# AIML-IfI/openset-imagenet

Measured on AMD Instinct MI355X. Metric: images/sec (whole node) ResNet-50 + entropic-open-set, Protocol 2, 1/2/4/8 GPUs, higher is better.
Workload: dtype f32; 1 GPU; Protocol 2, ResNet-50, entropic open-set loss, batch 128/GPU; workload_key=p2, classes=30, batch_per_gpu=128, global_batch=128, image=3x224x224, loss=entropic, optimizer=adam lr=1e-3, parallelism=dp1

## Files before the change

### openset-imagenet_amd/csrc/conv_wino.hip

```cpp
#include "conv_common.h"
#include <algorithm>
#include <type_traits>
#include <utility>

using namespace osi_conv;

namespace {

#ifndef OSI_WABL
#define OSI_WABL 0
#endif
#ifndef OSI_FABL
#define OSI_FABL 0
#endif
#ifndef OSI_STAGE_OUT
#define OSI_STAGE_OUT 1
#endif
#ifndef OSI_XSPREAD
#define OSI_XSPREAD 8
#endif
constexpr int KC = 16;
constexpr int PF = 6;

struct WinoP {
    const float* x;
    const float* u;
    float* y;
    const float* sc;
    const float* sh;
    int H, W, Kc, Nc, TH, TW, T, KS, CB, MT, NT;
    int x_bytes, y_bytes, u_bytes;
    float* pmean;
    float* pm2;
    int P;
    float cnt, rcnt;
    const float* ey0;
    const float *escale0, *eshift0, *emean0, *einv0;
    float* esum;
    const float *osc, *osh;
    int orelu;
    int q, r, nfull;
    float* slab;
    int slab_bytes;
};

__device__ __forceinline__ f32x2 pk_add(f32x2 a, f32x2 b) {
    f32x2 r;
    asm volatile("v_pk_add_f32 %0, %1, %2" : "=v"(r) : "v"(a), "v"(b));
    return r;
}
__device__ __forceinline__ f32x2 pk_sub(f32x2 a, f32x2 b) {
    f32x2 r;
    asm volatile("v_pk_add_f32 %0, %1, %2 neg_lo:[0,1] neg_hi:[0,1]" : "=v"(r) : "v"(a), "v"(b));
    return r;
}
__device__ __forceinline__ f32x2 pk_neg(f32x2 a) {
    f32x2 r;
    asm volatile("v_pk_add_f32 %0, 0, %1 neg_lo:[0,1] neg_hi:[0,1]" : "=v"(r) : "v"(a));
    return r;
}
__device__ __forceinline__ f32x2 pk_fma(f32x2 a, f32x2 b, f32x2 c) {
    f32x2 r;
    asm volatile("v_pk_fma_f32 %0, %1, %2, %3" : "=v"(r) : "v"(a), "v"(b), "v"(c));
    return r;
}
__device__ __forceinline__ f32x4 pk_add(f32x4 a, f32x4 b) {
    const f32x2 lo = pk_add(__builtin_shufflevector(a, a, 0, 1), __builtin_shufflevector(b, b, 0, 1));
    const f32x2 hi = pk_add(__builtin_shufflevector(a, a, 2, 3), __builtin_shufflevector(b, b, 2, 3));
    return __builtin_shufflevector(lo, hi, 0, 1, 2, 3);
}
__device__ __forceinline__ f32x4 pk_sub(f32x4 a, f32x4 b) {
    const f32x2 lo = pk_sub(__builtin_shufflevector(a, a, 0, 1), __builtin_shufflevector(b, b, 0, 1));
    const f32x2 hi = pk_sub(__builtin_shufflevector(a, a, 2, 3), __builtin_shufflevector(b, b, 2, 3));
    return __builtin_shufflevector(lo, hi, 0, 1, 2, 3);
}

template <class F, int... I>
__device__ __forceinline__ void for_each_const(F& f, std::integer_sequence<int, I...>) {
    (f(std::integral_constant<int, I>{}), ...);
}

__device__ __forceinline__ float row16_sum(float v) {
    v += __builtin_bit_cast(float, __builtin_amdgcn_update_dpp(0, __builtin_bit_cast(int, v), 0xB1, 0xF, 0xF, true));
    v += __builtin_bit_cast(float, __builtin_amdgcn_update_dpp(0, __builtin_bit_cast(int, v), 0x4E, 0xF, 0xF, true));
    v += __builtin_bit_cast(float, __builtin_amdgcn_update_dpp(0, __builtin_bit_cast(int, v), 0x141, 0xF, 0xF, true));
    v += __builtin_bit_cast(float, __builtin_amdgcn_update_dpp(0, __builtin_bit_cast(int, v), 0x140, 0xF, 0xF, true));
    return v;
}

template <int FLIP>
__global__ __launch_bounds__(256) void k_wino_weights(const float* __restrict__ w, float* __restrict__ u, int Kc, int Nc, int KS, int CB) {
    const int idx = blockIdx.x * 256 + threadIdx.x;
    const int K4 = Kc / 4;
    if (idx >= K4 * Nc) return;
    const int n = idx % Nc, k0 = (idx / Nc) * 4;
    f32x4 g[3][3];
#pragma unroll
    for (int r = 0; r < 3; ++r)
#pragma unroll
        for (int s = 0; s < 3; ++s) {
            if (FLIP) {
#pragma unroll
                for (int e = 0; e < 4; ++e) g[r][s][e] = w[((size_t)((k0 + e) * 3 + (2 - r)) * 3 + (2 - s)) * Nc + n];
            } else g[r][s] = ld4(w + ((size_t)(n * 3 + r) * 3 + s) * Kc + k0);
        }
    f32x4 t[4][3];
#pragma unroll
    for (int s = 0; s < 3; ++s) {
        t[0][s] = g[0][s];
        t[1][s] = 0.5f * (g[0][s] + g[1][s] + g[2][s]);
        t[2][s] = 0.5f * (g[0][s] - g[1][s] + g[2][s]);
        t[3][s] = g[2][s];
    }
    const int ks = k0 / KC, j = (k0 % KC) / 8, h = (k0 % 8) / 4, cb = n / 32, lane = h * 32 + n % 32;
#pragma unroll
    for (int xi = 0; xi < 4; ++xi) {
        f32x4 v[4];
        v[0] = t[xi][0];
        v[1] = 0.5f * (t[xi][0] + t[xi][1] + t[xi][2]);
        v[2] = 0.5f * (t[xi][0] - t[xi][1] + t[xi][2]);
        v[3] = t[xi][2];
#pragma unroll
        for (int nu = 0; nu < 4; ++nu) {
            const int p = xi * 4 + nu;
            *reinterpret_cast<f32x4*>(u + ((((size_t)(p * KS + ks) * CB + cb) * 2 + j) * 64 + lane) * 4) = v[nu];
        }
    }
}

struct Seg { int v, ks0, ks1, slot; bool valid; };

__device__ __forceinline__ void unit_of(int v, int MT, int NT, int& mt, int& nt) {
    const int full = (MT / 8) * 8 * NT;
    if (v < full) {
        const int xcd = v & 7, slot = v >> 3;
        nt = slot % NT;
        mt = (slot / NT) * 8 + xcd;
    } else {
        const int rem = MT & 7, vv = v - full;
        mt = (MT / 8) * 8 + vv % rem;
        nt = vv / rem;
    }
}
__device__ __forceinline__ int piece_begin(int w, int r, int KS, int G) { return (int)(((long)w * r * KS) / G); }

__device__ __forceinline__ Seg seg_phase2(int w, int q, int r, int KS, int G, bool second, int first_u) {
    Seg s{0, 0, 0, -1, false};
    if (r == 0) return s;
    const int b0 = piece_begin(w, r, KS, G), b1 = piece_begin(w + 1, r, KS, G);
    if (b1 <= b0) return s;
    const int u0 = b0 / KS;
    if (!second) {
        s.v = q * G + u0; s.ks0 = b0 - u0 * KS; s.ks1 = min(KS, s.ks0 + (b1 - b0)); s.slot = 0; s.valid = true;
        return s;
    }
    if (b1 > (u0 + 1) * KS) { s.v = q * G + u0 + 1; s.ks0 = 0; s.ks1 = b1 - (u0 + 1) * KS; s.slot = 1; s.valid = true; }
    return s;
}
__device__ __forceinline__ Seg seg_first(int w, int nfull, int q, int r, int KS, int G) {
    if (w < nfull) return Seg{w, 0, KS, -1, true};
    return seg_phase2(w, q, r, KS, G, false, 0);
}
__device__ __forceinline__ Seg seg_next(const Seg& c, int w, int nfull, int q, int r, int KS, int G) {
    if (c.slot < 0) {
        if (c.v + G < nfull) return Seg{c.v + G, 0, KS, -1, true};
        return seg_phase2(w, q, r, KS, G, false, 0);
    }
    if (c.slot == 0) return seg_phase2(w, q, r, KS, G, true, 0);
    return Seg{0, 0, 0, -1, false};
}

template <bool ODD, class PUT>
__device__ __forceinline__ void epi0_quad(const WinoP& p, PUT put, int g, f32x4 (&o)[4], const uint32_t (&po)[4], int ch0,
                                          int part, int lane) {
    {
#pragma unroll
        for (int k = 0; k < 4; ++k) put(k, g, o[k]);
        if (p.pmean) {
            f32x4 s1 = {0.f, 0.f, 0.f, 0.f};
#pragma unroll
            for (int k = 0; k < 4; ++k) {
                if constexpr (ODD) { if (po[k] == OOB) o[k] = f32x4{0.f, 0.f, 0.f, 0.f}; }
                s1 += o[k];
            }
            f32x4 mean, m2;
#pragma unroll
            for (int e = 0; e < 4; ++e) mean[e] = row16_sum(s1[e]) * p.rcnt;
            f32x4 s2 = {0.f, 0.f, 0.f, 0.f};
#pragma unroll
            for (int k = 0; k < 4; ++k) {
                const f32x4 dlt = o[k] - mean;
                s2 += dlt * dlt;
            }
#pragma unroll
            for (int e = 0; e < 4; ++e) {
                m2[e] = row16_sum(s2[e]);
                if constexpr (ODD) m2[e] -= (64.f - p.cnt) * mean[e] * mean[e];
            }
            if ((lane & 15) == 0 && part < p.P) {
                *reinterpret_cast<f32x4*>(p.pmean + (size_t)part * p.Nc + ch0 + 8 * g) = mean;
                *reinterpret_cast<f32x4*>(p.pm2 + (size_t)part * p.Nc + ch0 + 8 * g) = m2;
            }
        }
    }
}

template <class PUT>
__device__ __forceinline__ void epi2_quad(const WinoP& p, PUT put, int g, const f32x4 (&o)[4], const f32x4& sc, const f32x4& sh) {
// ... 218 lines not shown
                if constexpr (pos >= 8 && pos < 12) act_col(pos - 8, sc4, sh4);
                if constexpr (pos >= 12) row_store(pos - 12, buf ^ 1);
#endif
                b0 = nb0; b1 = nb1;
                __builtin_amdgcn_sched_barrier(0);
            };
            for_each_const(position, std::make_integer_sequence<int, 16>{});
            __syncthreads();
            buf ^= 1;
        }

        const int ch0 = CW * cur_nt + 32 * wm + 4 * hh;
        const int part = cur_mt * (TB / 16) + 2 * wn + ((lane >> 4) & 1);
        const __amdgpu_buffer_rsrc_t rs = make_rsrc(p.slab, p.slab_bytes);
        const __amdgpu_buffer_rsrc_t r0y = make_rsrc(EPI == 1 ? p.ey0 : p.y, p.y_bytes);
        Epi1Ops L1{};
        if constexpr (EPI == 1) { if (seg.slot < 0) L1 = epi1_load(p, r0y, 0, po, ch0); }
        float* const stage = WIDE ? sV + 2 * 16 * TB * KC : sV + (buf ^ 1) * (16 * TB * KC);
        if (seg.slot < 0 && wm == 0 && hh == 0) {
#pragma unroll
            for (int k = 0; k < 4; ++k) sPo[ntile * 4 + k] = po[k];
        }
#pragma unroll
        for (int g = (OSI_FABL & 16) ? 3 : 0; g < 4; ++g) {
            f32x4 o[4];
#pragma unroll
            for (int e = 0; e < 4; ++e) {
                const int r = 4 * g + e;
                float s[2][4];
#pragma unroll
                for (int nu = 0; nu < 4; ++nu) {
                    float m0, m1, m2, m3;
                    asm volatile("v_accvgpr_read_b32 %0, %1" : "=v"(m0) : "a"(acc[nu][r]));
                    asm volatile("v_accvgpr_read_b32 %0, %1" : "=v"(m1) : "a"(acc[4 + nu][r]));
                    asm volatile("v_accvgpr_read_b32 %0, %1" : "=v"(m2) : "a"(acc[8 + nu][r]));
                    asm volatile("v_accvgpr_read_b32 %0, %1" : "=v"(m3) : "a"(acc[12 + nu][r]));
                    s[0][nu] = m0 + m1 + m2;
                    s[1][nu] = m1 - m2 - m3;
                }
#pragma unroll
                for (int i = 0; i < 2; ++i) {
                    o[i * 2][e] = s[i][0] + s[i][1] + s[i][2];
                    o[i * 2 + 1][e] = s[i][1] - s[i][2] - s[i][3];
                }
            }
            if (seg.slot < 0) {
                auto put = [&](int k, int gq, const f32x4& v) {
#if OSI_STAGE_OUT
                    const int chunk = (32 * wm + 8 * gq + 4 * hh) >> 2;
                    *reinterpret_cast<f32x4*>(stage + (ntile * 4 + k) * CW + 4 * (chunk ^ (ntile & 15))) = v;
#else
                    bst4(ry, v, po[k] == OOB ? OOB : po[k] + 32u * gq, 0);
#endif
                };
                if constexpr (EPI == 0) epi0_quad<ODD>(p, put, g, o, po, ch0, part, lane);
                else if constexpr (EPI == 2) epi2_quad(p, put, g, o, ld4(p.osc + ch0 + 8 * g), ld4(p.osh + ch0 + 8 * g));
                else {
                    const Epi1Ops Ln = epi1_load(p, r0y, g < 3 ? g + 1 : 3, po, ch0);
                    epi1_apply<ODD>(p, put, g, o, po, ch0, part, lane, L1);
                    L1 = Ln;
                }
            } else {
                const uint32_t so = (uint32_t)((wg * 2 + seg.slot) * 65536 + ((wave * 4 + g) * 4) * 1024 + lane * 16);
#pragma unroll
                for (int k = 0; k < 4; ++k) bst4(rs, o[k], so + (uint32_t)k * 1024u, 0);
            }
        }
        if (OSI_STAGE_OUT && seg.slot < 0) {
            __syncthreads();
            constexpr int CPR = CW / 4, NCH = TB * 4 * CPR;
#pragma unroll 4
            for (int it = 0; it < NCH / 256; ++it) {
                const int idx = it * 256 + tid, row = idx / CPR, chunk = idx % CPR;
                const f32x4 v = *reinterpret_cast<const f32x4*>(stage + row * CW + 4 * (chunk ^ ((row >> 2) & 15)));
                const uint32_t base = sPo[row];
                bst4(ry, v, base == OOB ? OOB : base + (uint32_t)chunk * 16u, 0);
            }
            __syncthreads();
        }
        if (!nxt.valid) break;
        seg = nxt;
#pragma unroll
        for (int k = 0; k < 4; ++k) po[k] = po_next[k];
        ua = ua_next;
    }
}

template <int EPI, bool ODD, bool WIDE>
__global__ __launch_bounds__(64) void k_wino_fixup(WinoP p, int G) {
    const int lane = threadIdx.x, u = blockIdx.x >> 4, wave = (blockIdx.x >> 2) & 3, g = blockIdx.x & 3;
    const int wm = WIDE ? wave : wave >> 1, wn = WIDE ? 0 : wave & 1;
    const int ntile = 32 * wn + (lane & 31), hh = lane >> 5;
    int mt, nt;
    unit_of(p.q * G + u, p.MT, p.NT, mt, nt);
    uint32_t po[4];
    out_offsets<WIDE>(p, mt, nt, ntile, wm, hh, true, po);
    const __amdgpu_buffer_rsrc_t ry = make_rsrc(p.y, p.y_bytes);
    const __amdgpu_buffer_rsrc_t rs = make_rsrc(p.slab, p.slab_bytes);
    const int s0 = u * p.KS, s1 = s0 + p.KS;
    int w = (int)(((long)s0 * G) / ((long)p.r * p.KS));
    w = w > 0 ? w - 1 : 0;
    while (piece_begin(w + 1, p.r, p.KS, G) <= s0) ++w;
    f32x4 o[4] = {{0.f, 0.f, 0.f, 0.f}, {0.f, 0.f, 0.f, 0.f}, {0.f, 0.f, 0.f, 0.f}, {0.f, 0.f, 0.f, 0.f}};
    int b0 = piece_begin(w, p.r, p.KS, G);
    for (int ww = w; ww < G && b0 < s1; ++ww) {
        const int b1 = piece_begin(ww + 1, p.r, p.KS, G);
        if (b1 > b0) {
            const int slot = (b0 / p.KS == u) ? 0 : 1;
            const uint32_t so = (uint32_t)((ww * 2 + slot) * 65536 + ((wave * 4 + g) * 4) * 1024 + lane * 16);
#pragma unroll
            for (int k = 0; k < 4; ++k) o[k] += bld4(rs, so + (uint32_t)k * 1024u, 0);
        }
        b0 = b1;
    }
    const int ch0 = (WIDE ? 128 : 64) * nt + 32 * wm + 4 * hh, part = mt * (WIDE ? 2 : 4) + 2 * wn + ((lane >> 4) & 1);
    auto put = [&](int k, int gq, const f32x4& v) { bst4(ry, v, po[k] == OOB ? OOB : po[k] + 32u * gq, 0); };
    if constexpr (EPI == 0) epi0_quad<ODD>(p, put, g, o, po, ch0, part, lane);
    else if constexpr (EPI == 2) epi2_quad(p, put, g, o, ld4(p.osc + ch0 + 8 * g), ld4(p.osh + ch0 + 8 * g));
    else {
        const Epi1Ops L = epi1_load(p, make_rsrc(p.ey0, p.y_bytes), g, po, ch0);
        epi1_apply<ODD>(p, put, g, o, po, ch0, part, lane, L);
    }
}

struct WgradP {
    const float* x;
    const float* dy;
    float* slab;
    const float* sc;
    const float* sh;
    int H, W, Cin, Cout, TH, TW, T;
    int CBn, S, steps;
    int x_bytes, dy_bytes;
    FastDiv dTHW, dTW;
};

template <bool XF>
__global__ __launch_bounds__(512) void k_wino_wgrad(WgradP p) {
    __shared__ __attribute__((aligned(16))) float sL[2 * 2 * 16 * 2 * 64 * 4];
    const int tid = threadIdx.x, lane = tid & 63, hh = lane >> 5, l31 = lane & 31;
    const int wave = __builtin_amdgcn_readfirstlane(tid >> 6);
    const int ph = wave >> 2, wm = (wave >> 1) & 1, wn = wave & 1;
    const int item = blockIdx.x;
    const int split = item % p.S, blk = item / p.S, cb = blk % p.CBn, kb = blk / p.CBn;
    const int lh = wave & 1, kq = wave >> 1;
    const uint32_t xlane = (uint32_t)((cb * 64 + lane) * 4), dlane = (uint32_t)((kb * 64 + lane) * 4);
    const int t_first = split * p.steps * 8;
    const __amdgpu_buffer_rsrc_t rx = make_rsrc(p.x, p.x_bytes);
    const __amdgpu_buffer_rsrc_t rd = make_rsrc(p.dy, p.dy_bytes);
    float sc = 1.f, sh = 0.f;
    if constexpr (XF) { sc = p.sc[cb * 64 + lane]; sh = p.sh[cb * 64 + lane]; }
    const int cin4 = p.Cin * 4, cout4 = p.Cout * 4;

    float rx_[2][16], rd_[2][4];
    unsigned okx_[2], okd_[2];
    uint32_t srb[4], scb[4], sdr[2], sdc[2];
    auto prep_step = [&](int st, auto SETC) {
        constexpr int set = decltype(SETC)::value;
        const int t_raw = t_first + st * 8 + wave;
        const bool live = t_raw < p.T;
        const uint32_t t = (uint32_t)(live ? t_raw : p.T - 1);
        const uint32_t b = fdiv(t, p.dTHW), rem = t - b * p.dTHW.d, th = fdiv(rem, p.dTW), tw = rem - th * p.dTW.d;
        const int y0 = 2 * (int)th - 1, x0 = 2 * (int)tw - 1;
        unsigned rok = 0, cok = 0;
#pragma unroll
        for (int i = 0; i < 4; ++i) {
// ... 149 lines not shown
#pragma unroll
            for (int e = 0; e < 4; ++e) {
                const int r = 8 * PH + 4 * hq + e;
                const int m = 32 * wm + (r & 3) + 8 * (r >> 2) + 4 * hh;
                auto S = [&](int pos) { return (pos >> 3) == PH ? acc[pos & 7][r] : o[pos & 7][e]; };
                float t[3][4];
#pragma unroll
                for (int nu = 0; nu < 4; ++nu) {
                    const float s0 = S(nu), s1 = S(4 + nu), s2 = S(8 + nu), s3 = S(12 + nu);
                    t[0][nu] = s0 + 0.5f * (s1 + s2);
                    t[1][nu] = 0.5f * (s1 - s2);
                    t[2][nu] = 0.5f * (s1 + s2) + s3;
                }
#pragma unroll
                for (int rr = 0; rr < 3; ++rr) {
                    out[(size_t)((rr * 3 + 0) * 64 + m) * 64] = t[rr][0] + 0.5f * (t[rr][1] + t[rr][2]);
                    out[(size_t)((rr * 3 + 1) * 64 + m) * 64] = 0.5f * (t[rr][1] - t[rr][2]);
                    out[(size_t)((rr * 3 + 2) * 64 + m) * 64] = 0.5f * (t[rr][1] + t[rr][2]) + t[rr][3];
                }
            }
        }
    };
    if (ph == 0) finish(S0{}); else finish(S1{});
}

__global__ __launch_bounds__(256) void k_wino_wgrad_reduce(const float* __restrict__ slab, float* __restrict__ dw, int Cin, int Cout, int CBn, int S,
                                                           int SG) {
    __shared__ f32x4 part[256];
    const int per = 256 / SG;
    const int o = threadIdx.x % per, g = threadIdx.x / per;
    const int idx = blockIdx.x * per + o;
    const int C4 = Cin / 4, n = Cout * 9 * C4;
    f32x4 a = {0.f, 0.f, 0.f, 0.f};
    int k = 0, tap = 0, c4 = 0;
    if (idx < n) {
        c4 = idx % C4; tap = (idx / C4) % 9; k = idx / (C4 * 9);
        const int cb = (c4 * 4) / 64, kb = k / 64;
        const float* src = slab + (size_t)((kb * CBn + cb) * S) * (9 * 4096) + (size_t)(tap * 64 + (k & 63)) * 64 + ((c4 * 4) & 63);
        for (int s = g; s < S; s += SG) a += ld4(src + (size_t)s * (9 * 4096));
    }
    part[threadIdx.x] = a;
    __syncthreads();
    if (g == 0 && idx < n) {
        for (int j = 1; j < SG; ++j) a += part[j * per + o];
        *reinterpret_cast<f32x4*>(dw + ((size_t)k * 9 + tap) * Cin + c4 * 4) = a;
    }
}

int backward_exclusive_cus();
struct WgradPlan { int S, steps; size_t slab_floats; };
WgradPlan plan_wgrad_wino(const osi_conv_desc* d) {
    const int T = d->B * ((d->H + 1) / 2) * ((d->W + 1) / 2);
    const int blocks = (d->Cout / 64) * (d->Cin / 64);
    int G = backward_exclusive_cus();
    int S = G / blocks;
    if (S < 1) S = 1;
    const int max_s = (T + 63) / 64;
    if (S > max_s) S = max_s;
    const int per = (T + S - 1) / S;
    WgradPlan w;
    w.S = S; w.steps = (per + 7) / 8;
    w.slab_floats = (size_t)blocks * S * 9 * 4096;
    return w;
}

bool wino_shape(const osi_conv_desc* d) {
    return conv_desc_ok(d) && d->R == 3 && d->S == 3 && d->stride == 1 && d->pad == 1 && d->H == d->Ho && d->W == d->Wo && d->H >= 2 && d->W >= 2;
}

struct Geo { int TH, TW, T, MT, P; bool odd; float cnt; bool uniform; };
Geo geo_of(const osi_conv_desc* d) {
    Geo g{};
    g.TH = (d->H + 1) / 2; g.TW = (d->W + 1) / 2; g.T = d->B * g.TH * g.TW; g.MT = (g.T + 63) / 64; g.P = (g.T + 15) / 16;
    const bool even = d->H % 2 == 0 && d->W % 2 == 0;
    g.odd = !even || g.T % 64 != 0;
    const int thw = g.TH * g.TW;
    if (g.P == 1) { g.uniform = true; g.cnt = (float)((long)d->B * d->H * d->W); }
    else if (g.T % 16 == 0 && even) { g.uniform = true; g.cnt = 64.f; }
    else if (g.T % 16 == 0 && 16 % thw == 0) { g.uniform = true; g.cnt = (float)(16 / thw * d->H * d->W); }
    else { g.uniform = false; g.cnt = 64.f; }
    return g;
}

template <int FLIP>
int launch_weights(const float* w, float* u, int Kc, int Nc, hipStream_t st) {
    hipLaunchKernelGGL(k_wino_weights<FLIP>, dim3((unsigned)((Kc / 4 * Nc + 255) / 256)), dim3(256), 0, st, w, u, Kc, Nc, Kc / KC, Nc / 32);
    OSI_LAUNCH_CHECK();
    return OSI_OK;
}

bool wide_units(int Nc) { return g_osi_tuning.wino_wide && Nc % 128 == 0; }

WinoP make_wp(const osi_conv_desc* d, const Geo& g, int Kc, int Nc) {
    WinoP p{};
    const bool wide = wide_units(Nc);
    p.H = d->H; p.W = d->W; p.Kc = Kc; p.Nc = Nc; p.TH = g.TH; p.TW = g.TW; p.T = g.T; p.KS = Kc / KC; p.CB = Nc / 32;
    p.MT = wide ? (g.T + 31) / 32 : g.MT; p.NT = Nc / (wide ? 128 : 64);
    p.x_bytes = (int)((size_t)d->B * d->H * d->W * Kc * 4);
    p.y_bytes = (int)((size_t)d->B * d->H * d->W * Nc * 4);
    p.u_bytes = (int)((size_t)16 * Kc * Nc * 4);
    p.P = g.P; p.cnt = g.cnt; p.rcnt = 1.f / g.cnt;
    return p;
}

int backward_exclusive_cus() {
    if (g_osi_tuning.tail_cus > 0) return chip_cus();
    int res = 8 * g_osi_tuning.dp_reserved_cus;
    if (res > hw_cus() / 4) res = hw_cus() / 4;
    const int n = hw_cus() - res;
    return n < 8 ? 8 : n;
}
int wino_grid(bool backward) {
    int cus = backward ? backward_exclusive_cus() : chip_cus();
    if (cus > hw_cus()) cus = hw_cus();
    cus = cus / 8 * 8;
    return cus < 8 ? 8 : cus;
}
constexpr size_t SLOT_BYTES = 65536;
size_t u_bytes_of(const osi_conv_desc* d) { return ((size_t)16 * d->Cin * d->Cout * sizeof(float) + 255) / 256 * 256; }
size_t slab_bytes_of() { return (size_t)(hw_cus() / 8 * 8 < 8 ? 8 : hw_cus() / 8 * 8) * 2 * SLOT_BYTES; }

void plan_units(WinoP& p, void* slab, size_t slab_bytes, const osi_conv_desc* d, int G, bool input_gradient) {
    const int V = p.MT * p.NT;
    p.q = V / G; p.r = V - p.q * G; p.nfull = p.q * G;
    const bool heavy_tail = p.r > 0 && (double)(G - p.r) / (double)G / (double)(p.q + 1) >= 0.15;
    const int sk = g_osi_tuning.wino_streamk;
    const bool cut = sk == 1 || (sk == 2 && !input_gradient) || (sk == 3 && input_gradient);
    if (!cut || (p.KS <= 4 && !heavy_tail)) { p.nfull = V; p.r = 0; }
    p.slab = (float*)slab;
    p.slab_bytes = (int)std::min<size_t>(slab_bytes, (size_t)hw_cus() * 2 * SLOT_BYTES);
}

}

extern "C" {

int osi_conv_wino_eligible(const osi_conv_desc* d, int input_gradient) {
    if (!wino_shape(d)) return 0;
    const int Kc = input_gradient ? d->Cout : d->Cin, Nc = input_gradient ? d->Cin : d->Cout;
    if (Kc % KC || Nc % 64) return 0;
    const Geo g = geo_of(d);
    return (input_gradient || g.uniform) ? 1 : 0;
}

size_t osi_conv_wino_workspace(const osi_conv_desc* d) {
    if (!wino_shape(d)) return 0;
    return u_bytes_of(d) + slab_bytes_of();
}

static int fwd_wino_impl(const osi_conv_desc* d, const float* x, const float* in_scale, const float* in_shift, const float* w, float* u,
                         float* y, void* slab, size_t slab_bytes, float* pstats, size_t pstats_bytes, int* P, int* rows_per_block,
                         osi_stream_t stream, const osi_conv_epilogue* epi = nullptr) {
    OSI_REQUIRE(x && u && y && slab && osi_conv_wino_eligible(d, 0));
    OSI_REQUIRE(!epi || (epi->scale && epi->shift && !epi->residual && !in_scale && !pstats));
    OSI_REQUIRE((in_scale == nullptr) == (in_shift == nullptr));
    OSI_REQUIRE(slab_bytes >= slab_bytes_of());
    OSI_REQUIRE(!pstats || (P && rows_per_block));
    hipStream_t st = (hipStream_t)stream;
    const Geo g = geo_of(d);
    WinoP p = make_wp(d, g, d->Cin, d->Cout);
    p.x = x; p.u = u; p.y = y; p.sc = in_scale; p.sh = in_shift;
    if (epi) { p.osc = epi->scale; p.osh = epi->shift; p.orelu = epi->relu ? 1 : 0; }
    if (pstats) {
        OSI_REQUIRE(pstats_bytes >= (size_t)2 * g.P * d->Cout * sizeof(float));
        p.pmean = pstats; p.pm2 = pstats + (size_t)g.P * d->Cout;
        *P = g.P; *rows_per_block = (int)g.cnt;
    }
    if (w) { if (int e = launch_weights<0>(w, u, d->Cin, d->Cout, st)) return e; }
    const int G = wino_grid(false);
    OSI_REQUIRE(slab_bytes >= (size_t)G * 2 * SLOT_BYTES);
    plan_units(p, slab, slab_bytes, d, G, false);
    const dim3 grid((unsigned)G), blk(256);
    const bool wide = wide_units(d->Cout), odd = g.odd || (wide && g.T % 32 != 0);
    auto launch = [&](auto XFC, auto ODDC, auto WIDEC) {
        constexpr bool xf = decltype(XFC)::value, od = decltype(ODDC)::value, wd = decltype(WIDEC)::value;
        hipLaunchKernelGGL((k_wino<xf, 0, od, wd>), grid, blk, 0, st, p);
        if (hipGetLastError() != hipSuccess) return OSI_ERR_LAUNCH;
        if (p.r > 0) {
            hipLaunchKernelGGL((k_wino_fixup<0, od, wd>), dim3((unsigned)p.r * 16), dim3(64), 0, st, p, G);
            if (hipGetLastError() != hipSuccess) return OSI_ERR_LAUNCH;
        }
        return OSI_OK;
    };
    auto launch_epi = [&](auto ODDC, auto WIDEC) {
        constexpr bool od = decltype(ODDC)::value, wd = decltype(WIDEC)::value;
        hipLaunchKernelGGL((k_wino<false, 2, od, wd>), grid, blk, 0, st, p);
        if (hipGetLastError() != hipSuccess) return OSI_ERR_LAUNCH;
        if (p.r > 0) {
            hipLaunchKernelGGL((k_wino_fixup<2, od, wd>), dim3((unsigned)p.r * 16), dim3(64), 0, st, p, G);
            if (hipGetLastError() != hipSuccess) return OSI_ERR_LAUNCH;
        }
        return OSI_OK;
    };
    using T_ = std::true_type; using F_ = std::false_type;
    if (epi) {
        if (odd) return wide ? launch_epi(T_{}, T_{}) : launch_epi(T_{}, F_{});
        return wide ? launch_epi(F_{}, T_{}) : launch_epi(F_{}, F_{});
    }
    const int sel = (in_scale ? 4 : 0) | (odd ? 2 : 0) | (wide ? 1 : 0);
    switch (sel) {
        case 0: return launch(F_{}, F_{}, F_{});
        case 1: return launch(F_{}, F_{}, T_{});
        case 2: return launch(F_{}, T_{}, F_{});
        case 3: return launch(F_{}, T_{}, T_{});
        case 4: return launch(T_{}, F_{}, F_{});
        case 5: return launch(T_{}, F_{}, T_{});
        case 6: return launch(T_{}, T_{}, F_{});
        default: return launch(T_{}, T_{}, T_{});
    }
}

int osi_conv_fwd_wino(const osi_conv_desc* d, const float* x, const float* in_scale, const float* in_shift, const float* w, float* y,
                      void* ws, size_t ws_bytes, float* pstats, size_t pstats_bytes, int* P, int* rows_per_block, osi_stream_t stream) {
    OSI_REQUIRE(w && ws && wino_shape(d) && ws_bytes >= osi_conv_wino_workspace(d));
    return fwd_wino_impl(d, x, in_scale, in_shift, w, (float*)ws, y, (char*)ws + u_bytes_of(d), ws_bytes - u_bytes_of(d), pstats, pstats_bytes, P,
                         rows_per_block, stream);
}

size_t osi_conv_wino_weights_bytes(const osi_conv_desc* d) { return wino_shape(d) ? u_bytes_of(d) : 0; }
size_t osi_conv_wino_slab_bytes(void) { return slab_bytes_of(); }
int osi_conv_wino_transform_weights(const osi_conv_desc* d, const float* w, int input_gradient, float* u, size_t u_bytes, osi_stream_t stream) {
    OSI_REQUIRE(w && u && osi_conv_wino_eligible(d, input_gradient ? 1 : 0) && u_bytes >= u_bytes_of(d));
    return input_gradient ? launch_weights<1>(w, u, d->Cout, d->Cin, (hipStream_t)stream) : launch_weights<0>(w, u, d->Cin, d->Cout, (hipStream_t)stream);
}
int osi_conv_fwd_wino_pre(const osi_conv_desc* d, const float* x, const float* in_scale, const float* in_shift, const float* u, float* y,
                          void* slab, size_t slab_bytes, float* pstats, size_t pstats_bytes, int* P, int* rows_per_block, osi_stream_t stream) {
    return fwd_wino_impl(d, x, in_scale, in_shift, nullptr, const_cast<float*>(u), y, slab, slab_bytes, pstats, pstats_bytes, P, rows_per_block, stream);
}

int osi_conv_fwd_wino_epilogue_pre(const osi_conv_desc* d, const float* x, const float* u, float* out, const osi_conv_epilogue* e, void* slab,
                                   size_t slab_bytes, osi_stream_t stream) {
    OSI_REQUIRE(e);
    return fwd_wino_impl(d, x, nullptr, nullptr, nullptr, const_cast<float*>(u), out, slab, slab_bytes, nullptr, 0, nullptr, nullptr, stream, e);
}

static int dgrad_wino_impl(const osi_conv_desc* d, const float* dy, const float* w, float* u, float* dx, const osi_dgrad_fusion* f, void* slab,
                           size_t slab_bytes, int* P, osi_stream_t stream) {
    OSI_REQUIRE(dy && u && dx && slab && f && P && osi_conv_wino_eligible(d, 1));
    OSI_REQUIRE(!f->relu_mask && !f->y1 && !f->pool_idx && f->addend_stride != 2);
    OSI_REQUIRE(f->y0 && f->scale0 && f->shift0);
    OSI_REQUIRE(!f->partials || (f->mean0 && f->invstd0));
    OSI_REQUIRE(slab_bytes >= slab_bytes_of());
    hipStream_t st = (hipStream_t)stream;
    const Geo g = geo_of(d);
    WinoP p = make_wp(d, g, d->Cout, d->Cin);
    p.x = dy; p.u = u; p.y = dx;
    p.ey0 = f->y0; p.escale0 = f->scale0; p.eshift0 = f->shift0;
    p.emean0 = f->mean0 ? f->mean0 : f->scale0; p.einv0 = f->invstd0 ? f->invstd0 : f->scale0;
    if (f->partials) {
        OSI_REQUIRE(f->partials_bytes >= (size_t)3 * g.P * d->Cin * sizeof(float));
        p.esum = f->partials;
    }
    *P = g.P;
    if (w) { if (int e = launch_weights<1>(w, u, d->Cout, d->Cin, st)) return e; }
    const int G = wino_grid(true);
    OSI_REQUIRE(slab_bytes >= (size_t)G * 2 * SLOT_BYTES);
    plan_units(p, slab, slab_bytes, d, G, true);
    const dim3 grid((unsigned)G), blk(256);
    const bool wide = wide_units(d->Cin), odd = g.odd || (wide && g.T % 32 != 0);
    auto launch = [&](auto ODDC, auto WIDEC) {
        constexpr bool od = decltype(ODDC)::value, wd = decltype(WIDEC)::value;
        hipLaunchKernelGGL((k_wino<false, 1, od, wd>), grid, blk, 0, st, p);
        if (hipGetLastError() != hipSuccess) return OSI_ERR_LAUNCH;
        if (p.r > 0) {
            hipLaunchKernelGGL((k_wino_fixup<1, od, wd>), dim3((unsigned)p.r * 16), dim3(64), 0, st, p, G);
            if (hipGetLastError() != hipSuccess) return OSI_ERR_LAUNCH;
        }
        return OSI_OK;
    };
    using T_ = std::true_type; using F_ = std::false_type;
    if (odd) return wide ? launch(T_{}, T_{}) : launch(T_{}, F_{});
    return wide ? launch(F_{}, T_{}) : launch(F_{}, F_{});
}

int osi_conv_dgrad_fused_wino(const osi_conv_desc* d, const float* dy, const float* w, float* dx, const osi_dgrad_fusion* f, void* ws,
                              size_t ws_bytes, int* P, osi_stream_t stream) {
    OSI_REQUIRE(w && ws && wino_shape(d) && ws_bytes >= osi_conv_wino_workspace(d));
    return dgrad_wino_impl(d, dy, w, (float*)ws, dx, f, (char*)ws + u_bytes_of(d), ws_bytes - u_bytes_of(d), P, stream);
}
int osi_conv_dgrad_fused_wino_pre(const osi_conv_desc* d, const float* dy, const float* u, float* dx, const osi_dgrad_fusion* f, void* slab,
                                  size_t slab_bytes, int* P, osi_stream_t stream) {
    return dgrad_wino_impl(d, dy, nullptr, const_cast<float*>(u), dx, f, slab, slab_bytes, P, stream);
}

size_t osi_conv_wgrad_wino_workspace(const osi_conv_desc* d) {
    if (!wino_shape(d) || d->Cin % 64 || d->Cout % 64) return 0;
    return plan_wgrad_wino(d).slab_floats * sizeof(float);
}

int osi_conv_wgrad_wino(const osi_conv_desc* d, const float* dy, const float* x, const float* in_scale, const float* in_shift, float* dw,
                        void* ws, size_t ws_bytes, osi_stream_t stream) {
    OSI_REQUIRE(dy && x && dw && ws && wino_shape(d) && d->Cin % 64 == 0 && d->Cout % 64 == 0);
    OSI_REQUIRE((in_scale == nullptr) == (in_shift == nullptr));
    const WgradPlan w = plan_wgrad_wino(d);
    OSI_REQUIRE(ws_bytes >= w.slab_floats * sizeof(float));
    hipStream_t st = (hipStream_t)stream;
    WgradP p{};
    p.x = x; p.dy = dy; p.slab = (float*)ws; p.sc = in_scale; p.sh = in_shift;
    p.H = d->H; p.W = d->W; p.Cin = d->Cin; p.Cout = d->Cout; p.TH = (d->H + 1) / 2; p.TW = (d->W + 1) / 2; p.T = d->B * p.TH * p.TW;
    p.CBn = d->Cin / 64; p.S = w.S; p.steps = w.steps;
    p.dTHW = make_fastdiv((uint32_t)(p.TH * p.TW)); p.dTW = make_fastdiv((uint32_t)p.TW);
    p.x_bytes = (int)((size_t)d->B * d->H * d->W * d->Cin * 4);
    p.dy_bytes = (int)((size_t)d->B * d->H * d->W * d->Cout * 4);
    const dim3 grid((unsigned)((d->Cout / 64) * p.CBn * p.S)), blk(256);
    if (in_scale) hipLaunchKernelGGL((k_wino_wgrad<true>), grid, dim3(512), 0, st, p);
    else hipLaunchKernelGGL((k_wino_wgrad<false>), grid, dim3(512), 0, st, p);
    OSI_LAUNCH_CHECK();
    const int n = d->Cout * 9 * (d->Cin / 4);
    int SG = 1;
    while (SG * 2 <= p.S && SG < 16) SG *= 2;
    const int per = 256 / SG;
    hipLaunchKernelGGL(k_wino_wgrad_reduce, dim3((unsigned)((n + per - 1) / per)), blk, 0, st, (const float*)ws, dw, d->Cin, d->Cout, p.CBn, p.S, SG);
    OSI_LAUNCH_CHECK();
    return OSI_OK;
}

}
```

Baseline: 4502 images/sec.

## Add 512-thread two-wave Winograd kernel with new weight layout for 64-channel convs

Adds k_wino2, a 512-thread Winograd F(2,3) kernel that splits each 64-tile unit across eight waves. It uses 16x16x4 MFMAs, a reshuffled weight-fragment layout (slice_channel) and a shallower U prefetch depth. It is selected when the channel count is not a multiple of 128, as in ResNet-50's 64-channel 3x3 layers. The aim is more waves per unit and better latency hiding for narrow layers, at the cost of more shared memory and registers per block and a dependence on the weight transform and the existing fixup path matching the new layout.

```diff
diff --git a/openset-imagenet_amd/csrc/conv_wino.hip b/openset-imagenet_amd/csrc/conv_wino.hip
--- a/openset-imagenet_amd/csrc/conv_wino.hip
+++ b/openset-imagenet_amd/csrc/conv_wino.hip
@@ -21,6 +21,7 @@
 #endif
 constexpr int KC = 16;
 constexpr int PF = 6;
+constexpr int PF2 = 3;
 
 struct WinoP {
     const float* x;
@@ -88,12 +89,17 @@
     return v;
 }
 
-template <int FLIP>
+__host__ __device__ constexpr int slice_channel(int m, int kg) { return 8 * (m >> 1) + 2 * (m & 1) + 4 * (kg & 1) + (kg >> 1); }
+
+template <int FLIP, bool TWO>
 __global__ __launch_bounds__(256) void k_wino_weights(const float* __restrict__ w, float* __restrict__ u, int Kc, int Nc, int KS, int CB) {
     const int idx = blockIdx.x * 256 + threadIdx.x;
     const int K4 = Kc / 4;
     if (idx >= K4 * Nc) return;
     const int n = idx % Nc, k0 = (idx / Nc) * 4;
+    int kk[4];
+#pragma unroll
+    for (int e = 0; e < 4; ++e) kk[e] = TWO ? (k0 / KC) * KC + slice_channel(e, (k0 % KC) / 4) : k0 + e;
     f32x4 g[3][3];
 #pragma unroll
     for (int r = 0; r < 3; ++r)
@@ -101,7 +107,10 @@
         for (int s = 0; s < 3; ++s) {
             if (FLIP) {
 #pragma unroll
-                for (int e = 0; e < 4; ++e) g[r][s][e] = w[((size_t)((k0 + e) * 3 + (2 - r)) * 3 + (2 - s)) * Nc + n];
+                for (int e = 0; e < 4; ++e) g[r][s][e] = w[((size_t)(kk[e] * 3 + (2 - r)) * 3 + (2 - s)) * Nc + n];
+            } else if (TWO) {
+#pragma unroll
+                for (int e = 0; e < 4; ++e) g[r][s][e] = w[((size_t)(n * 3 + r) * 3 + s) * Kc + kk[e]];
             } else g[r][s] = ld4(w + ((size_t)(n * 3 + r) * 3 + s) * Kc + k0);
         }
     f32x4 t[4][3];
@@ -113,6 +122,7 @@
         t[3][s] = g[2][s];
     }
     const int ks = k0 / KC, j = (k0 % KC) / 8, h = (k0 % 8) / 4, cb = n / 32, lane = h * 32 + n % 32;
+    const size_t frag = TWO ? ((size_t)(n / 16) * 64 + ((k0 % KC) / 4) * 16 + n % 16) * 4 : (((size_t)cb * 2 + j) * 64 + lane) * 4;
 #pragma unroll
     for (int xi = 0; xi < 4; ++xi) {
         f32x4 v[4];
@@ -123,7 +133,7 @@
 #pragma unroll
         for (int nu = 0; nu < 4; ++nu) {
             const int p = xi * 4 + nu;
-            *reinterpret_cast<f32x4*>(u + ((((size_t)(p * KS + ks) * CB + cb) * 2 + j) * 64 + lane) * 4) = v[nu];
+            *reinterpret_cast<f32x4*>(u + (size_t)(p * KS + ks) * (16 * Nc) + frag) = v[nu];
         }
     }
 }
@@ -508,6 +518,242 @@
         seg = nxt;
 #pragma unroll
         for (int k = 0; k < 4; ++k) po[k] = po_next[k];
+        ua = ua_next;
+    }
+}
+
+template <bool XF, int EPI, bool ODD>
+__global__ __launch_bounds__(512) void k_wino2(WinoP p) {
+    constexpr int TB = 64, CW = 64, NV = 2, TPT = KC / NV;
+    __shared__ __attribute__((aligned(16))) float sV[2 * 16 * TB * KC];
+    __shared__ uint32_t sPo[256];
+    const int tid = threadIdx.x, lane = tid & 63, wave = __builtin_amdgcn_readfirstlane(tid >> 6);
+    const int th = wave & 1, c16 = wave >> 1;
+    const int tl = lane & 15, kg = lane >> 4;
+    const __amdgpu_buffer_rsrc_t rx = make_rsrc(p.x, p.x_bytes);
+    const __amdgpu_buffer_rsrc_t ry = make_rsrc(p.y, p.y_bytes);
+    const __amdgpu_buffer_rsrc_t ru = make_rsrc(p.u, p.u_bytes);
+    const int G = gridDim.x, wg = blockIdx.x;
+    const int ltile = tid / TPT, q = tid % TPT;
+    const int ntile0 = 32 * th + tl;
+    const int THW = p.TH * p.TW;
+
+    Seg seg = seg_first(wg, p.nfull, p.q, p.r, p.KS, G);
+    if (!seg.valid) return;
+    int mt, nt;
+    unit_of(seg.v, p.MT, p.NT, mt, nt);
+
+    uint32_t off0[4], off1[4];
+    bool rowok[4], colok[4];
+    uint32_t ua, ua_next;
+    const uint32_t colstep = (uint32_t)p.Kc * 4;
+    auto setup = [&](int mt_, int nt_, bool live, uint32_t& ua_) {
+        const int t = mt_ * TB + ltile;
+        const int b = t / THW, rem = t - b * THW, thh = rem / p.TW, tw = rem - thh * p.TW;
+        const uint32_t base = (uint32_t)((((b * p.H + 2 * thh - 1) * p.W + 2 * tw) * p.Kc + q * NV) * 4);
+#pragma unroll
+        for (int j = 0; j < 4; ++j) colok[j] = (unsigned)(2 * tw - 1 + j) < (unsigned)p.W;
+#pragma unroll
+        for (int i = 0; i < 4; ++i) {
+            rowok[i] = live && t < p.T && (unsigned)(2 * thh - 1 + i) < (unsigned)p.H;
+            const uint32_t o1 = base + (uint32_t)(i * p.W) * colstep;
+            off1[i] = rowok[i] ? o1 : OOB;
+            off0[i] = rowok[i] && colok[0] ? o1 - colstep : OOB;
+        }
+        ua_ = (uint32_t)((((CW / 16) * nt_ + c16) * 64 + lane) * 16);
+    };
+    setup(mt, nt, true, ua);
+    float* wb[NV];
+#pragma unroll
+    for (int e = 0; e < NV; ++e) {
+        const int c = q * NV + e, ckg = ((c >> 2) & 1) | ((c & 1) << 1), cm = ((c >> 1) & 1) | ((c >> 3) << 1);
+        wb[e] = sV + ltile * KC + 4 * (ckg ^ ((ltile >> 2) & 3)) + cm;
+    }
+    const float* const rb = sV + ntile0 * KC + 4 * (kg ^ ((ntile0 >> 2) & 3));
+    const uint32_t ustep = (uint32_t)p.Nc * 64;
+
+    f32x4acc acc[16][2];
+    using XT = f32x2;
+    XT xr[16];
+    auto load_x1 = [&](int ks, int k) {
+        const int i = k >> 2, j = k & 3;
+        const uint32_t voff = j == 0 ? off0[i] : j == 1 ? off1[i] : colok[j] ? off1[i] : OOB;
+        const uint32_t soff = (uint32_t)ks * (KC * 4) + (j >= 2 ? (uint32_t)(j - 1) * colstep : 0u);
+        xr[k] = __builtin_bit_cast(f32x2, __builtin_amdgcn_raw_buffer_load_b64(rx, voff, soff, 0));
+    };
+    auto add = [](XT a, XT b) { return pk_add(a, b); };
+    auto sub = [](XT a, XT b) { return pk_sub(a, b); };
+    float scv[NV], shv[NV];
+    auto act_col = [&](int j) {
+        if constexpr (XF) {
+#pragma unroll
+            for (int i = 0; i < 4; ++i) {
+                const unsigned long long okm = __builtin_amdgcn_ballot_w64(rowok[i] && colok[j]);
+#pragma unroll
+                for (int e = 0; e < NV; ++e)
+                    asm volatile("v_fma_f32 %0, %0, %1, %2\n\tv_max_f32 %0, 0, %0\n\tv_cndmask_b32 %0, 0, %0, %3"
+                                 : "+v"(xr[i * 4 + j][e]) : "v"(scv[e]), "v"(shv[e]), "s"(okm));
+            }
+        }
+        const XT d0 = xr[j], d1 = xr[4 + j], d2 = xr[8 + j], d3 = xr[12 + j];
+        xr[j] = sub(d0, d2); xr[4 + j] = add(d1, d2); xr[8 + j] = sub(d2, d1); xr[12 + j] = sub(d1, d3);
+    };
+    auto row_store = [&](int i, int buf) {
+        const int o0 = buf * (16 * TB * KC) + (i * 4) * (TB * KC);
+        const XT t0 = xr[i * 4], t1 = xr[i * 4 + 1], t2 = xr[i * 4 + 2], t3 = xr[i * 4 + 3];
+        const XT o[4] = {sub(t0, t2), add(t1, t2), sub(t2, t1), sub(t1, t3)};
+#pragma unroll
+        for (int nu = 0; nu < 4; ++nu) {
+            wb[0][o0 + nu * (TB * KC)] = o[nu][0]; wb[1][o0 + nu * (TB * KC)] = o[nu][1];
+        }
+    };
+    auto ld_scale = [&](int ks) {
+        if constexpr (XF) {
+#pragma unroll
+            for (int e = 0; e < NV; ++e) { scv[e] = p.sc[ks * KC + q * NV + e]; shv[e] = p.sh[ks * KC + q * NV + e]; }
+        }
+    };
+
+#pragma unroll
+    for (int e = 0; e < NV; ++e) { scv[e] = 1.f; shv[e] = 0.f; }
+#pragma unroll
+    for (int k = 0; k < 16; ++k) load_x1(seg.ks0, k);
+    ld_scale(seg.ks0);
+#pragma unroll
+    for (int j = 0; j < 4; ++j) act_col(j);
+#pragma unroll
+    for (int i = 0; i < 4; ++i) row_store(i, 0);
+
+    f32x4 a[16];
+    auto load_u = [&](int pos, uint32_t base, int ks) {
+        const uint32_t soff = (OSI_FABL & 1) ? 0u : (uint32_t)(pos * p.KS + ks) * ustep;
+        a[pos] = bld4(ru, base, soff);
+    };
+#pragma unroll
+    for (int i = 0; i < PF2; ++i) load_u(i, ua, seg.ks0);
+    __syncthreads();
+
+    int buf = 0;
+    for (;;) {
+#pragma unroll
+        for (int i = 0; i < 16; ++i)
+#pragma unroll
+            for (int tg = 0; tg < 2; ++tg) acc[i][tg] = f32x4acc{0.f, 0.f, 0.f, 0.f};
+        Seg nxt{0, 0, 0, -1, false};
+        const int cur_mt = mt, cur_nt = nt;
+        for (int ks = seg.ks0; ks < seg.ks1; ++ks) {
+            const bool last = ks + 1 == seg.ks1;
+            int ksn = ks + 1;
+            uint32_t uan = ua;
+            if (last) {
+                nxt = seg_next(seg, wg, p.nfull, p.q, p.r, p.KS, G);
+                if (nxt.valid) unit_of(nxt.v, p.MT, p.NT, mt, nt);
+                setup(mt, nt, nxt.valid, ua_next);
+                ksn = nxt.valid ? nxt.ks0 : 0;
+                uan = nxt.valid ? ua_next : ua;
+            }
+            ld_scale(ksn);
+            const float* r0 = rb + buf * (16 * TB * KC);
+            f32x4 b0 = *reinterpret_cast<const f32x4*>(r0), b1 = *reinterpret_cast<const f32x4*>(r0 + 16 * KC);
+            __builtin_amdgcn_sched_barrier(0);
+            auto position = [&](auto POSC) {
+                constexpr int pos = decltype(POSC)::value;
+                if (pos + PF2 < 16) load_u(pos + PF2, ua, ks);
+                else load_u(pos + PF2 - 16, uan, ksn);
+#if !(OSI_FABL & 2)
+                if constexpr (pos < 8) { load_x1(ksn, 2 * pos); load_x1(ksn, 2 * pos + 1); }
+#endif
+                f32x4 nb0 = b0, nb1 = b1;
+                if (pos < 15 && !(OSI_FABL & 8)) {
+                    nb0 = *reinterpret_cast<const f32x4*>(r0 + (pos + 1) * (TB * KC));
+                    nb1 = *reinterpret_cast<const f32x4*>(r0 + (pos + 1) * (TB * KC) + 16 * KC);
+                }
+                const f32x4 av = a[pos];
+#pragma unroll
+                for (int m = 0; m < 4; ++m) {
+                    acc[pos][0] = __builtin_amdgcn_mfma_f32_16x16x4f32(av[m], b0[m], acc[pos][0], 0, 0, 0);
+                    acc[pos][1] = __builtin_amdgcn_mfma_f32_16x16x4f32(av[m], b1[m], acc[pos][1], 0, 0, 0);
+                }
+#if !(OSI_FABL & 4)
+                if constexpr (pos >= 8 && pos < 12) act_col(pos - 8);
+                if constexpr (pos >= 12) row_store(pos - 12, buf ^ 1);
+#endif
+                b0 = nb0; b1 = nb1;
+                __builtin_amdgcn_sched_barrier(0);
+            };
+            for_each_const(position, std::make_integer_sequence<int, 16>{});
+            __syncthreads();
+            buf ^= 1;
+        }
+
+        const int chl = 16 * c16 + 4 * kg;
+        const int ch0 = CW * cur_nt + chl;
+        const __amdgpu_buffer_rsrc_t rs = make_rsrc(p.slab, p.slab_bytes);
+        const __amdgpu_buffer_rsrc_t r0y = make_rsrc(EPI == 1 ? p.ey0 : p.y, p.y_bytes);
+        uint32_t po[2][4];
+#pragma unroll
+        for (int tg = 0; tg < 2; ++tg) out_offsets<false>(p, cur_mt, cur_nt, ntile0 + 16 * tg, 0, chl >> 2, true, po[tg]);
+        Epi1Ops L1{};
+        if constexpr (EPI == 1) { if (seg.slot < 0) L1 = epi1_load(p, r0y, 0, po[0], ch0); }
+        float* const stage = sV + (buf ^ 1) * (16 * TB * KC);
+        if (seg.slot < 0 && chl == 0) {
+#pragma unroll
+            for (int tg = 0; tg < 2; ++tg)
+#pragma unroll
+                for (int k = 0; k < 4; ++k) sPo[(ntile0 + 16 * tg) * 4 + k] = po[tg][k];
+        }
+#pragma unroll
+        for (int tg = (OSI_FABL & 16) ? 1 : 0; tg < 2; ++tg) {
+            const int ntile = ntile0 + 16 * tg;
+            const int part = cur_mt * (TB / 16) + 2 * th + tg;
+            f32x4 o[4];
+#pragma unroll
+            for (int e = 0; e < 4; ++e) {
+                float s[2][4];
+#pragma unroll
+                for (int nu = 0; nu < 4; ++nu) {
+                    const float m0 = acc[nu][tg][e], m1 = acc[4 + nu][tg][e], m2 = acc[8 + nu][tg][e], m3 = acc[12 + nu][tg][e];
+                    s[0][nu] = m0 + m1 + m2;
+                    s[1][nu] = m1 - m2 - m3;
+                }
+#pragma unroll
+                for (int i = 0; i < 2; ++i) {
+                    o[i * 2][e] = s[i][0] + s[i][1] + s[i][2];
+                    o[i * 2 + 1][e] = s[i][1] - s[i][2] - s[i][3];
+                }
+            }
+            if (seg.slot < 0) {
+                auto put = [&](int k, int, const f32x4& v) {
+                    *reinterpret_cast<f32x4*>(stage + (ntile * 4 + k) * CW + 4 * ((chl >> 2) ^ (ntile & 15))) = v;
+                };
+                if constexpr (EPI == 0) epi0_quad<ODD>(p, put, 0, o, po[tg], ch0, part, lane);
+                else if constexpr (EPI == 2) epi2_quad(p, put, 0, o, ld4(p.osc + ch0), ld4(p.osh + ch0));
+                else {
+                    const Epi1Ops Ln = epi1_load(p, r0y, 0, po[1], ch0);
+                    epi1_apply<ODD>(p, put, 0, o, po[tg], ch0, part, lane, L1);
+                    L1 = Ln;
+                }
+            } else {
+                const int ow = (c16 >> 1) * 2 + th, og = 2 * (c16 & 1) + (kg >> 1), ol = 32 * (kg & 1) + 16 * tg + tl;
+                const uint32_t so = (uint32_t)((wg * 2 + seg.slot) * 65536 + ((ow * 4 + og) * 4) * 1024 + ol * 16);
+#pragma unroll
+                for (int k = 0; k < 4; ++k) bst4(rs, o[k], so + (uint32_t)k * 1024u, 0);
+            }
+        }
+        if (seg.slot < 0) {
+            __syncthreads();
+            constexpr int CPR = CW / 4, NCH = TB * 4 * CPR;
+#pragma unroll 4
+            for (int it = 0; it < NCH / 512; ++it) {
+                const int idx = it * 512 + tid, row = idx / CPR, chunk = idx % CPR;
+                const f32x4 v = *reinterpret_cast<const f32x4*>(stage + row * CW + 4 * (chunk ^ ((row >> 2) & 15)));
+                const uint32_t base = sPo[row];
+                bst4(ry, v, base == OOB ? OOB : base + (uint32_t)chunk * 16u, 0);
+            }
+            __syncthreads();
+        }
+        if (!nxt.valid) break;
+        seg = nxt;
         ua = ua_next;
     }
 }
@@ -823,14 +1069,22 @@
     return g;
 }
 
+bool wide_units(int Nc) { return g_osi_tuning.wino_wide && Nc % 128 == 0; }
+
+#ifdef OSI_WINO_ONE_WAVE
+bool two_wave(int Nc) { return false; }
+#else
+bool two_wave(int Nc) { return Nc % 128 != 0; }
+#endif
+
 template <int FLIP>
 int launch_weights(const float* w, float* u, int Kc, int Nc, hipStream_t st) {
-    hipLaunchKernelGGL(k_wino_weights<FLIP>, dim3((unsigned)((Kc / 4 * Nc + 255) / 256)), dim3(256), 0, st, w, u, Kc, Nc, Kc / KC, Nc / 32);
+    const dim3 grid((unsigned)((Kc / 4 * Nc + 255) / 256));
+    if (two_wave(Nc)) hipLaunchKernelGGL((k_wino_weights<FLIP, true>), grid, dim3(256), 0, st, w, u, Kc, Nc, Kc / KC, Nc / 32);
+    else hipLaunchKernelGGL((k_wino_weights<FLIP, false>), grid, dim3(256), 0, st, w, u, Kc, Nc, Kc / KC, Nc / 32);
     OSI_LAUNCH_CHECK();
     return OSI_OK;
 }
-
-bool wide_units(int Nc) { return g_osi_tuning.wino_wide && Nc % 128 == 0; }
 
 WinoP make_wp(const osi_conv_desc* d, const Geo& g, int Kc, int Nc) {
     WinoP p{};
@@ -911,11 +1165,14 @@
     const int G = wino_grid(false);
     OSI_REQUIRE(slab_bytes >= (size_t)G * 2 * SLOT_BYTES);
     plan_units(p, slab, slab_bytes, d, G, false);
-    const dim3 grid((unsigned)G), blk(256);
+    const bool two = two_wave(d->Cout);
+    const dim3 grid((unsigned)G), blk(two ? 512 : 256);
     const bool wide = wide_units(d->Cout), odd = g.odd || (wide && g.T % 32 != 0);
     auto launch = [&](auto XFC, auto ODDC, auto WIDEC) {
         constexpr bool xf = decltype(XFC)::value, od = decltype(ODDC)::value, wd = decltype(WIDEC)::value;
-        hipLaunchKernelGGL((k_wino<xf, 0, od, wd>), grid, blk, 0, st, p);
+        bool launched = false;
+        if constexpr (!wd) { if (two) { hipLaunchKernelGGL((k_wino2<xf, 0, od>), grid, blk, 0, st, p); launched = true; } }
+        if (!launched) hipLaunchKernelGGL((k_wino<xf, 0, od, wd>), grid, blk, 0, st, p);
         if (hipGetLastError() != hipSuccess) return OSI_ERR_LAUNCH;
         if (p.r > 0) {
             hipLaunchKernelGGL((k_wino_fixup<0, od, wd>), dim3((unsigned)p.r * 16), dim3(64), 0, st, p, G);
@@ -925,7 +1182,9 @@
     };
     auto launch_epi = [&](auto ODDC, auto WIDEC) {
         constexpr bool od = decltype(ODDC)::value, wd = decltype(WIDEC)::value;
-        hipLaunchKernelGGL((k_wino<false, 2, od, wd>), grid, blk, 0, st, p);
+        bool launched = false;
+        if constexpr (!wd) { if (two) { hipLaunchKernelGGL((k_wino2<false, 2, od>), grid, blk, 0, st, p); launched = true; } }
+        if (!launched) hipLaunchKernelGGL((k_wino<false, 2, od, wd>), grid, blk, 0, st, p);
         if (hipGetLastError() != hipSuccess) return OSI_ERR_LAUNCH;
         if (p.r > 0) {
             hipLaunchKernelGGL((k_wino_fixup<2, od, wd>), dim3((unsigned)p.r * 16), dim3(64), 0, st, p, G);
@@ -997,11 +1256,14 @@
     const int G = wino_grid(true);
     OSI_REQUIRE(slab_bytes >= (size_t)G * 2 * SLOT_BYTES);
     plan_units(p, slab, slab_bytes, d, G, true);
-    const dim3 grid((unsigned)G), blk(256);
+    const bool two = two_wave(d->Cin);
+    const dim3 grid((unsigned)G), blk(two ? 512 : 256);
     const bool wide = wide_units(d->Cin), odd = g.odd || (wide && g.T % 32 != 0);
     auto launch = [&](auto ODDC, auto WIDEC) {
         constexpr bool od = decltype(ODDC)::value, wd = decltype(WIDEC)::value;
-        hipLaunchKernelGGL((k_wino<false, 1, od, wd>), grid, blk, 0, st, p);
+        bool launched = false;
+        if constexpr (!wd) { if (two) { hipLaunchKernelGGL((k_wino2<false, 1, od>), grid, blk, 0, st, p); launched = true; } }
+        if (!launched) hipLaunchKernelGGL((k_wino<false, 1, od, wd>), grid, blk, 0, st, p);
         if (hipGetLastError() != hipSuccess) return OSI_ERR_LAUNCH;
         if (p.r > 0) {
             hipLaunchKernelGGL((k_wino_fixup<1, od, wd>), dim3((unsigned)p.r * 16), dim3(64), 0, st, p, G);
```

Measured after the change: 4517 images/sec, median of 6. About the same (+0.3%).
